# MarcoPolo/drand

Measured on AMD Instinct MI355X. Metric: verified beacons/sec (whole node), quicknet G1 scheme, higher is better.
Workload: dtype u32 (Fp products on 14x28-bit limbs, 64-bit MAD accumulators; 12x32-bit Montgomery storage); 1 GPU; bls-unchained-g1-rfc9380 batch verify of a 1048576-round chain, 1048576 rounds per GPU; scheme=bls-unchained-g1-rfc9380, rounds_total=1048576, rounds_per_gpu=1048576, global_batch=1048576, parallelism=round-shard x1

## Files before the change

### drand_amd/_lib.py

```python
import ctypes
import os

HERE = os.path.dirname(os.path.abspath(__file__))
LIB_PATH = os.environ.get("DRANDHIP_LIB") or os.path.join(HERE, "libdrandhip.so")

DH_OK = 0
DH_EINVAL = -1
DH_EDEVICE = -2
DH_ENOMEM = -3
DH_EKEY = -4
DH_ERECOVER = -5
DH_EBUSY = -6
DH_EABANDONED = -7
DH_ECORRUPT = -8
DH_ENOBEACON = -9
DH_NODE_CHECKED = 2
DH_DEFERRED = 1
DH_STORE_TRIMMED, DH_STORE_UNTRIMMED, DH_STORE_AUTO = 0, 1, 2

_c = ctypes
_P = _c.c_void_p
SIGNATURES = {
    "dh_init": (_c.c_int, [_c.c_uint32]),
    "dh_shutdown": (None, []),
    "dh_scheme_from_name": (_c.c_int, [_c.c_char_p]),
    "dh_sig_len": (_c.c_int, [_c.c_int]),
    "dh_key_len": (_c.c_int, [_c.c_int]),
    "dh_verify_batch": (_c.c_int, [_c.c_int, _c.c_char_p, _c.c_size_t, _P, _P, _c.c_size_t, _P, _c.c_size_t, _P,
                                   _c.c_size_t, _P, _P, _c.c_uint64]),
    "dh_verify_batch_device": (_c.c_int, [_c.c_int, _c.c_char_p, _c.c_size_t, _P, _P, _c.c_size_t, _P, _c.c_size_t,
                                          _P, _c.c_size_t, _P, _P, _c.c_uint64, _P, _P]),
    "dh_verify_beacon": (_c.c_int, [_c.c_int, _c.c_char_p, _c.c_size_t, _c.c_uint64, _c.c_char_p, _c.c_size_t,
                                    _c.c_char_p, _c.c_size_t]),
    "dh_verify_recovered": (_c.c_int, [_c.c_int, _c.c_char_p, _c.c_size_t, _c.c_char_p, _c.c_char_p, _c.c_size_t]),
    "dh_verify_recovered_batch": (_c.c_int, [_c.c_int, _c.c_char_p, _c.c_size_t, _P, _P, _c.c_size_t, _c.c_size_t, _P,
                                             _c.c_uint64]),
    "dh_digest_batch": (_c.c_int, [_c.c_int, _P, _P, _c.c_size_t, _P, _c.c_size_t, _P]),
    "dh_randomness_batch": (_c.c_int, [_c.c_int, _P, _c.c_size_t, _c.c_size_t, _P]),
    "dh_recover_batch": (_c.c_int, [_c.c_int, _c.c_char_p, _c.c_int, _c.c_int, _P, _P, _P, _c.c_size_t, _P, _P]),
    "dh_verify_partials_batch": (_c.c_int, [_c.c_int, _c.c_char_p, _c.c_int, _c.c_int, _P, _P, _P, _c.c_size_t, _P]),
    "dh_bls_verify_batch": (_c.c_int, [_c.c_int, _P, _c.c_size_t, _P, _P, _P, _P, _c.c_size_t, _c.c_size_t, _P, _P,
                                       _c.c_uint64, _P]),
    "dh_identity_hash_batch": (_c.c_int, [_c.c_int, _P, _c.c_size_t, _P]),
    "dh_identity_verify_batch": (_c.c_int, [_c.c_int, _P, _P, _c.c_size_t, _c.c_size_t, _P]),
    "dh_schnorr_verify_batch": (_c.c_int, [_c.c_int, _P, _c.c_size_t, _P, _P, _P, _P, _c.c_size_t, _c.c_size_t, _P, _P]),
    "dh_schnorr_sig_len": (_c.c_int, [_c.c_int]),
    "dh_sign_batch": (_c.c_int, [_c.c_int, _c.c_char_p, _P, _P, _c.c_size_t, _P, _c.c_size_t, _P]),
    "dh_public_key": (_c.c_int, [_c.c_int, _c.c_char_p, _P]),
    "dh_partial_bytes": (_c.c_int, [_c.c_int]),
    "dh_set_split": (_c.c_int, [_c.c_uint64, _c.c_int]),
    "dh_hash_to_curve": (_c.c_int, [_c.c_int, _P, _P, _c.c_size_t, _c.c_char_p, _c.c_size_t, _P]),
    "dh_batch_begin": (_c.c_int, [_c.c_int, _c.c_char_p, _c.c_size_t, _P, _P, _c.c_size_t, _P, _c.c_size_t, _P,
                                  _c.c_size_t, _P, _P, _c.c_uint64, _P, _c.POINTER(_P), _P]),
    "dh_batch_check": (_c.c_int, [_P, _P, _c.c_size_t, _P]),
    "dh_batch_stream": (_P, [_P]),
    "dh_check_partials": (_c.c_int, [_c.c_int, _c.c_char_p, _c.c_size_t, _P, _c.c_size_t, _c.POINTER(_c.c_int)]),
    "dh_batch_finish": (_c.c_int, [_P, _c.c_int, _P]),
    "dh_bolt_index": (_c.c_int, [_P, _c.c_size_t, _P, _P, _c.c_size_t, _P]),
    "dh_store_open_bolt": (_c.c_int, [_P, _c.c_size_t, _c.POINTER(_P)]),
    "dh_store_stat": (_c.c_int, [_P, _P]),
    "dh_store_columns_device": (_c.c_int, [_P, _c.c_uint64, _c.c_uint64, _c.c_size_t, _P, _P, _P, _c.c_size_t, _P, _P,
                                           _c.c_size_t, _P, _P]),
    "dh_store_check_past": (_c.c_int, [_P, _c.c_int, _c.c_char_p, _c.c_size_t, _c.c_uint64, _c.c_size_t, _c.c_uint64, _P,
                                       _c.c_size_t, _P, _P, _P]),
    "dh_store_close": (None, [_P]),
    "dh_store_open_bolt_format": (_c.c_int, [_P, _c.c_size_t, _c.c_int, _c.POINTER(_P)]),
    "dh_store_format_stat": (_c.c_int, [_P, _P]),
    "dh_store_beacons_device": (_c.c_int, [_P, _c.c_uint64, _c.c_uint64, _c.c_size_t, _c.c_size_t, _P, _P, _P, _P, _P, _P,
                                           _c.c_size_t, _P, _P, _c.c_size_t, _P, _P]),
    "dh_store_deferred": (_c.c_int, [_P, _c.c_uint64, _c.c_uint64, _P, _c.c_size_t, _P]),
    "dh_profile": (_c.c_int, [_c.c_int]),
    "dh_profile_read": (_c.c_int, [_c.c_char_p, _c.c_size_t]),
    "dh_last_error_string": (_c.c_char_p, []),
    "dh_version": (_c.c_char_p, []),
}

_lib = None


class LibraryMissing(RuntimeError):
    pass


def load():
# ... 18 lines not shown
```

### drand_amd/csrc/codec.hpp

```cpp
#pragma once
#include "h2c.hpp"
#include "fp28.hpp"
#include "fp2_28.hpp"

namespace dh {

enum : uint8_t { DEC_OK = 1, DEC_INF = 2, DEC_BAD = 0 };

DH_DEV bool fp_lex_gt_half(const fp& mont_y) { return int_gt_half_p(fp_from_mont(mont_y)); }

DH_DEV bool fp2_lex_largest(const fp2& y) {
  fp c0 = fp_from_mont(y.c0), c1 = fp_from_mont(y.c1);
  return fp_is_zero(c1) ? int_gt_half_p(c0) : int_gt_half_p(c1);
}

DH_DEV void be48_words(uint32_t out[12], const uint8_t* in, bool mask_flags) {
#pragma unroll
  for (int i = 0; i < 12; i++) {
    uint32_t w = __builtin_bswap32(*(const uint32_t*)(in + 44 - 4 * i));
    out[i] = w;
  }
  if (mask_flags) out[11] &= 0x1fffffffu;
}

DH_DEV bool g1_in_subgroup(const aff<fp>& p) {
  return g1_in_subgroup28([&] { return p; });
}

DH_DEV bool g2_in_subgroup(const aff<fp2>& p) {
  return g2_in_subgroup28(p);
}

DH_DEV uint8_t g1_decompress(aff<fp>& out, const uint8_t* b, bool subgroup) {
  uint32_t w[12];
  be48_words(w, b, false);
  const uint32_t flags = w[11] >> 29;
  if (!(flags & 4)) return DEC_BAD;
  w[11] &= 0x1fffffffu;
  if (flags & 2) {
    uint32_t nz = flags & 1;
#pragma unroll
    for (int i = 0; i < 12; i++) nz |= w[i];
    return nz ? DEC_BAD : DEC_INF;
  }
  if (!int_lt_p(w)) return DEC_BAD;
  fp x;
#pragma unroll
  for (int i = 0; i < 12; i++) x.v[i] = w[i];
  x = fp_to_mont(x);
  fp rhs = fp_add(fp_mul(fp_sqr(x), x), fp_c(cst::B1));
  fp y;
  if (!fp_sqrt(y, rhs)) return DEC_BAD;
  if (fp_lex_gt_half(y) != (bool)(flags & 1)) y = fp_neg(y);
  out.x = x;
  out.y = y;
  if (subgroup && !g1_in_subgroup(out)) return DEC_BAD;
  return DEC_OK;
}

DH_DEV uint8_t g2_decompress(aff<fp2>& out, const uint8_t* b, bool subgroup) {
  uint32_t w1[12], w0[12];
  be48_words(w1, b, false);
  be48_words(w0, b + 48, false);
  const uint32_t flags = w1[11] >> 29;
  if (!(flags & 4)) return DEC_BAD;
  w1[11] &= 0x1fffffffu;
  if (flags & 2) {
    uint32_t nz = flags & 1;
#pragma unroll
    for (int i = 0; i < 12; i++) nz |= w1[i] | w0[i];
    return nz ? DEC_BAD : DEC_INF;
  }
  if (!int_lt_p(w0) || !int_lt_p(w1)) return DEC_BAD;
  fp2 x;
#pragma unroll
  for (int i = 0; i < 12; i++) {
    x.c0.v[i] = w0[i];
    x.c1.v[i] = w1[i];
  }
  x.c0 = fp_to_mont(x.c0);
  x.c1 = fp_to_mont(x.c1);
  fp2 rhs = fp2_add(fp2_mul(fp2_sqr(x), x), fp2_c(cst::B2));
  fp2 y;
  if (!fp2_sqrt(y, rhs)) return DEC_BAD;
  if (fp2_lex_largest(y) != (bool)(flags & 1)) y = fp2_neg(y);
  out.x = x;
  out.y = y;
  if (subgroup && !g2_in_subgroup(out)) return DEC_BAD;
  return DEC_OK;
// ... 36 lines not shown
```

### drand_amd/csrc/drandhip.cpp

```cpp
#include <hip/hip_runtime.h>
#include <stdarg.h>
#include <stdio.h>
#include <string.h>
#include <sys/random.h>

#include <algorithm>
#include <atomic>
#include <condition_variable>
#include <cmath>
#include <functional>
#include <map>
#include <memory>
#include <chrono>
#include <mutex>
#include <string>
#include <thread>
#include <vector>

#include "../../include/drandhip.h"
#include "bolt.hpp"
#include "kernels.hpp"

namespace {

// ... 711 lines not shown
static bool subgroup_batch_on() {
  static const bool v = [] {
    const char* e = getenv("DRANDHIP_SUBGROUP_BATCH");
    return !(e && e[0] == '0');
  }();
  return v;
}
static size_t sub_batch_min() {
  static const size_t v = [] {
    const char* e = getenv("DRANDHIP_SUB_BATCH_MIN");
    const long long d = e ? atoll(e) : 0;
    return (size_t)(d >= 1 ? d : 131072);
  }();
  return v;
}
constexpr size_t SUB_BATCH_MIN_G2_DEFAULT = 393216;
static size_t sub_batch_min_g2() {
  static const size_t v = [] {
    const char* e = getenv("DRANDHIP_SUB_BATCH_MIN_G2");
    const long long d = e ? atoll(e) : 0;
    return (size_t)(d >= 1 ? d : SUB_BATCH_MIN_G2_DEFAULT);
  }();
  return v;
}
static int sub_backoff() {
  static const int v = [] {
    const char* e = getenv("DRANDHIP_SUB_BACKOFF");
    const long d = e ? atol(e) : -1;
    return (int)(d >= 0 && d <= 1 << 20 ? d : 15);
  }();
  return v;
}

static int msm_workspace(worker* w, const dh::msm_geom& g, size_t m, size_t ngroups, size_t jw, dh::msm_ws& ws,
                         bool sub = false, bool g2 = false) {
  const size_t nk = ngroups * g.nwin * (size_t)g.nbuck;
  HIP_TRY(w->cnt.ensure(nk * 4));
  HIP_TRY(w->off.ensure((nk + 1) * 4));
  HIP_TRY(w->scan_tmp.ensure(((nk + 4095) / 4096 + 1) * 4));
  HIP_TRY(w->list.ensure(dh::msm_entries(g, m) * 4));
  HIP_TRY(w->buckets.ensure(2 * nk * jw * 4));
  const size_t segs_bytes = 2 * ngroups * g.nwin * g.nseg * jw * 4;
  HIP_TRY(w->segs.ensure(2 * segs_bytes));
  HIP_TRY(w->outA.ensure(ngroups * jw * 4));
  HIP_TRY(w->outB.ensure(ngroups * jw * 4));
  HIP_TRY(w->out2.ensure(2 * ngroups * jw * 4));
  HIP_TRY(w->pass.ensure(ngroups));
  HIP_TRY(w->part.ensure(dh::msm_part_bytes(dh::msm_entries(g, m), jw, 2)));
  HIP_TRY(w->meta.ensure(dh::msm_meta_bytes(dh::msm_entries(g, m))));
  ws = dh::msm_ws{w->cnt.as<uint32_t>(), w->off.as<uint32_t>(), w->scan_tmp.as<uint32_t>(), w->list.as<uint32_t>(),
                  w->buckets.as<uint32_t>(), w->segs.as<uint32_t>(), w->out2.as<uint32_t>(), w->part.as<uint32_t>(),
                  w->meta.as<uint32_t>(), 0, (uint32_t*)((uint8_t*)w->segs.p + segs_bytes)};
  if (sub) {
    HIP_TRY(w->sub_tmp.ensure(dh::sub_batch_tmp_bytes(g2, g)));
    HIP_TRY(w->sub_pass.ensure(8));
    ws.sub = w->sub_tmp.as<uint32_t>();
  }
  return DH_OK;
}

int verify_core(worker* w, int scheme, const uint8_t* pk, size_t pk_len, const uint64_t* d_rounds, const uint8_t* d_sigs,
                size_t sig_stride, const uint8_t* d_prevs, size_t prev_stride, const uint32_t* d_prev_lens, size_t n,
                uint8_t* d_verdict, uint8_t* d_rand, uint64_t seed, hipStream_t st, uint64_t* stats,
                const uint8_t* d_msgs32 = nullptr, int mode = VM_FULL, prep_gate* gate = nullptr) {
  const bool g2 = sig_on_g2(scheme);
  const int sig_len = g2 ? 96 : 48, key_len = g2 ? 48 : 96;
// ... 13 lines not shown
                            subgroup_batch_on();
  const bool sub_batch = sub_eligible && w->sub_fused_left == 0;
  if (sub_eligible && w->sub_fused_left > 0) w->sub_fused_left--;
  const int parts = g2 && !sub_batch ? 4 : 2;
  if (n >= ((size_t)1 << 31) / parts) return fail(DH_EINVAL, "batch too large");
  dh::msm_geom g0{};
  dh::msm_ws ws0{};
  if (mode <= VM_BEGIN) {
    int rc = ensure_key(w, g2, pk, pk_len, st);
    if (rc) return rc;

    HIP_TRY(w->status.ensure(n));
    HIP_TRY(w->sig_aff.ensure(n * aw * 4));
    HIP_TRY(w->q_pts.ensure(n * jw * 4));
    HIP_TRY(w->scal.ensure(n * 16));
    HIP_TRY(w->entries.ensure(n * 4));
    uint32_t seedw[8];
    rc = make_seed(seed, seedw);
    if (rc) return rc;
    uint32_t* d_seed = (uint32_t*)((uint8_t*)w->key_ok.p + 32);
    presorted = w->tail && st == w->stream && !skip0 && !one_stream;
    if (presorted) {
      hipStream_t ts = w->tail;
      HIP_TRY(hipMemcpyAsync(d_seed, seedw, 32, hipMemcpyHostToDevice, ts));
      HIP_TRY(dh::launch_scalars(d_seed, n, nullptr, w->scal.as<uint4>(), parts, ts));
      HIP_TRY(dh::launch_iota(w->entries.as<uint32_t>(), n, ts));
      g0 = geom_for(n, parts);
      g0.half_stride = (uint32_t)n;
      rc = msm_workspace(w, g0, n, 1, wsw, ws0, sub_batch, g2);
      if (rc) return rc;
      HIP_TRY(dh::launch_msm_sort(g0, w->entries.as<uint32_t>(), nullptr, nullptr, n, 1, w->scal.as<uint4>(), ws0, ts));
    }
    if (gate && gate->wait) HIP_TRY(hipStreamWaitEvent(st, gate->wait, 0));
    HIP_TRY(T.run(g2 ? "k_prep_sig<fp2>" : "k_prep_sig<fp>", [&] {
      return dh::launch_prep(g2, d_sigs, sig_stride, n, w->status.as<uint8_t>(), w->sig_aff.as<uint32_t>(), d_rand, st,
                             sub_batch);
    }));
    HIP_TRY(w->h2c_tmp.ensure(dh::hash_tmp_bytes(g2, n)));
    HIP_TRY(T.run(d_msgs32 ? (g2 ? "k_prep_msg32<fp2>" : "k_prep_msg32<fp>") : (g2 ? "k_prep_msg<fp2>" : "k_prep_msg<fp>"), [&] {
      return dh::launch_hash(g2, d_rounds, d_prevs, prev_stride, d_prev_lens, d_msgs32, n,
                             scheme == DH_SCHEME_CHAINED && d_prevs && !d_msgs32 ? 1 : 0, dst_id(scheme), w->status.as<uint8_t>(),
                             w->q_pts.as<uint32_t>(), w->h2c_tmp.as<uint32_t>(), st);
    }));
    if (!presorted) {
      HIP_TRY(hipMemcpyAsync(d_seed, seedw, 32, hipMemcpyHostToDevice, st));
      HIP_TRY(dh::launch_scalars(d_seed, n, w->status.as<uint8_t>(), w->scal.as<uint4>(), parts, st));
    }
    HIP_TRY(w->s28.ensure(parts * n * (g2 ? 64 : 32) * 4));
    HIP_TRY(w->q28.ensure(parts * n * (g2 ? 64 : 32) * 4));
    HIP_TRY(T.run(g2 ? "k_msm_prep28<fp2>" : "k_msm_prep28<fp>", [&] {
      return dh::launch_msm_prep28(g2, n, w->status.as<uint8_t>(), w->sig_aff.as<uint32_t>(), w->q_pts.as<uint32_t>(),
                                   w->s28.as<uint32_t>(), w->q28.as<uint32_t>(), st, 3, parts);
    }));
    HIP_TRY(hipMemsetAsync(d_verdict, 0, n, st));
    if (gate) {
      HIP_TRY(hipEventRecord(gate->done, st));
      gate->recorded();
    }
    if (mode == VM_FULL && w->tail && st == w->stream && !one_stream && prep_sync()) HIP_TRY(hipStreamSynchronize(st));
    if (!presorted) HIP_TRY(dh::launch_iota(w->entries.as<uint32_t>(), n, st));
  }
  if (w->tail && st == w->stream && !one_stream) {
    if (mode <= VM_BEGIN) {
      HIP_TRY(hipEventRecord(w->handoff, st));
      HIP_TRY(hipStreamWaitEvent(w->tail, w->handoff, 0));
    }
    st = w->tail;
    T.st = st;
  }

  size_t m = n;
  static const char* const msm_names[8] = {"msm_level0", "msm_bisect1", "msm_bisect2", "msm_bisect3",
                                           "msm_bisect4", "msm_bisect5", "msm_bisect6", "msm_bisect7+"};
  static const char* const chk_names[8] = {"k_group_check_level0", "k_group_check_bisect1", "k_group_check_bisect2",
                                           "k_group_check_bisect3", "k_group_check_bisect4", "k_group_check_bisect5",
                                           "k_group_check_bisect6", "k_group_check_bisect7+"};
// ... 1522 lines not shown
  if (n == 0) return DH_OK;
  size_t maxm = 0;
  for (size_t i = 0; i < n; i++) {
    if (msg_off[i + 1] < msg_off[i]) return fail(DH_EINVAL, "msg_off must be non-decreasing");
    maxm = std::max<size_t>(maxm, msg_off[i + 1] - msg_off[i]);
  }
  const size_t total = msg_off[n] - msg_off[0];
  const size_t stride = (64 + maxm + 4 + dst_len + 63) & ~(size_t)63;
  const size_t outlen = group == 1 ? 48 : 96;
  std::vector<uint32_t> off(n + 1);
  for (size_t i = 0; i <= n; i++) off[i] = msg_off[i] - msg_off[0];
  lease L;
  if (L.rc) return L.rc;
  worker* w = L.w;
  int rc = set_device_and_stream(w);
  if (rc) return rc;
  hipStream_t st = w->stream;
  HIP_TRY(w->in_sigs.ensure(total + 4));
  HIP_TRY(w->in_prev_lens.ensure((n + 1) * 4));
  HIP_TRY(w->key_raw.ensure(256));
  HIP_TRY(w->h2c_tmp.ensure(n * stride));
  HIP_TRY(w->out_rand.ensure(n * outlen));
  if (total) HIP_TRY(hipMemcpyAsync(w->in_sigs.p, msgs + msg_off[0], total, hipMemcpyHostToDevice, st));
  HIP_TRY(hipMemcpyAsync(w->in_prev_lens.p, off.data(), (n + 1) * 4, hipMemcpyHostToDevice, st));
  HIP_TRY(hipMemcpyAsync(w->key_raw.p, dst, dst_len, hipMemcpyHostToDevice, st));
  HIP_TRY(dh::launch_h2c_generic(group == 2, w->in_sigs.as<uint8_t>(), w->in_prev_lens.as<uint32_t>(), n,
                                 w->key_raw.as<uint8_t>(), (uint32_t)dst_len, w->h2c_tmp.as<uint8_t>(), stride,
                                 w->out_rand.as<uint8_t>(), st));
  HIP_TRY(hipMemcpyAsync(out, w->out_rand.p, n * outlen, hipMemcpyDeviceToHost, st));
  HIP_TRY(hipStreamSynchronize(st));
  return DH_OK;
}

int dh_public_key(int scheme, const uint8_t* sk32, uint8_t* key_out) {
  int kl = dh_key_len(scheme);
  if (kl < 0) return kl;
  if (!sk32 || !key_out) return fail(DH_EINVAL, "null argument");
  lease L;
  if (L.rc) return L.rc;
  worker* w = L.w;
  int rc = set_device_and_stream(w);
  if (rc) return rc;
  hipStream_t st = w->stream;
  uint32_t skw[8];
  sk_words(sk32, skw);
  HIP_TRY(w->key_ok.ensure(64));
  HIP_TRY(w->key_raw.ensure(96));
  HIP_TRY(hipMemcpyAsync(w->key_ok.p, skw, 32, hipMemcpyHostToDevice, st));
  HIP_TRY(dh::launch_pubkey(kl == 96, w->key_ok.as<uint32_t>(), w->key_raw.as<uint8_t>(), st));
  HIP_TRY(hipMemcpyAsync(key_out, w->key_raw.p, kl, hipMemcpyDeviceToHost, st));
  HIP_TRY(hipStreamSynchronize(st));
  return DH_OK;
}

}


static size_t store_max_bytes() {
  const char* e = getenv("DRANDHIP_STORE_MAX_BYTES");
  const long long v = e ? atoll(e) : 0;
  return v > 0 ? (size_t)v : (size_t)16 << 30;
}

struct prof_wall {
  const char* name;
  std::chrono::steady_clock::time_point t0;
// ... 647 lines not shown
```

### drand_amd/csrc/h2c.hpp

```cpp
#pragma once
#include "curve.hpp"
#include "sha256.hpp"
#include "fp28.hpp"

namespace dh {

DH_DEV fp fp_from_be512(const uint32_t hi[8], const uint32_t lo[8]) {
  fp h, l;
#pragma unroll
  for (int k = 0; k < 8; k++) {
    h.v[k] = hi[7 - k];
    l.v[k] = lo[7 - k];
  }
#pragma unroll
  for (int k = 8; k < 12; k++) h.v[k] = l.v[k] = 0;
  return fp_add(fp_mul(h, fp_c(cst::K256R)), fp_mul(l, fp_c(cst::R2)));
}

DH_DEV bool fp_sqrt_ratio(fp& y, const fp& u, const fp& v) {
  fp tv1 = fp_sqr(v);
  fp tv2 = fp_mul(u, v);
  tv1 = fp_mul(tv1, tv2);
  fp y1 = fp_pow_sched(tv1, cst::SCHED_SR1_C1, cst::SCHED_SR1_C1_LEN);
  y1 = fp_mul(y1, tv2);
// ... 64 lines not shown
  r.x = f_mul(s.xn, s.xd);
  r.y = f_mul(s.y, f_mul(f_sqr(s.xd), s.xd));
  return r;
}

template <class F>
DH_DEV bool jac_add_distinct(jac<F>& r, const jac<F>& p, const jac<F>& q) {
  F z1z1 = f_sqr(p.z);
  F z2z2 = f_sqr(q.z);
  F u1 = f_mul(p.x, z2z2);
  F u2 = f_mul(q.x, z1z1);
  F s1 = f_mul(f_mul(p.y, q.z), z2z2);
  F s2 = f_mul(f_mul(q.y, p.z), z1z1);
  F h = f_sub(u2, u1);
  if (f_is_zero(h)) return false;
  F rr = f_dbl(f_sub(s2, s1));
  F i = f_sqr(f_dbl(h));
  F j = f_mul(h, i);
  F v = f_mul(u1, i);
  r.x = f_sub(f_sub(f_sqr(rr), j), f_dbl(v));
  r.y = f_sub(f_mul(rr, f_sub(v, r.x)), f_dbl(f_mul(s1, j)));
  r.z = f_mul(f_sub(f_sub(f_sqr(f_add(p.z, q.z)), z1z1), z2z2), h);
  return true;
}

DH_DEV jac<fp> h2c_g1_map(const fp& u0, const fp& u1) {
  const jac<fp> p0 = swu_jac(sswu_g1(u0));
  const jac<fp> p1 = swu_jac(sswu_g1(u1));
  jac<fp> s;
  if (jac_add_distinct(s, p0, p1)) return iso11_jac(s);
  return jac_add(iso11_jac(p0), iso11_jac(p1));
}

DH_DEV jac<fp> h2c_g1_noclear(const sha_h& digest, int dst_id) {
  uint32_t b[4][8];
  xmd32<4>(b, digest, dst_id);
  return h2c_g1_map(fp_from_be512(b[0], b[1]), fp_from_be512(b[2], b[3]));
}

DH_DEV jac<fp> h2c_clear_g1(const jac<fp>& p) { return jac_add(jac_mul_uabs_j(p), p); }

DH_DEV swu_out<fp2> sswu_g2(const fp2& u) {
  const fp2 A = fp2_c(cst::SSWU2_A), B = fp2_c(cst::SSWU2_B), Z = fp2_c(cst::SSWU2_Z);
  fp2 tv1 = fp2_mul(Z, fp2_sqr(u));
  fp2 tv2 = fp2_add(fp2_sqr(tv1), tv1);
  fp2 tv3 = fp2_mul(B, fp2_add(tv2, fp2_one()));
  fp2 tv4 = fp2_mul(A, fp2_select(fp2_is_zero(tv2), Z, fp2_neg(tv2)));
  fp2 t2 = fp2_sqr(tv3);
  fp2 tv6 = fp2_sqr(tv4);
  t2 = fp2_add(t2, fp2_mul(A, tv6));
  t2 = fp2_mul(t2, tv3);
  tv6 = fp2_mul(tv6, tv4);
  t2 = fp2_add(t2, fp2_mul(B, tv6));
  fp2 x = fp2_mul(tv1, tv3);
  fp2 y1;
  bool gx1_sq = fp2_sqrt_ratio_cm(y1, t2, tv6);
  fp2 y = fp2_mul(fp2_mul(tv1, u), y1);
  x = fp2_select(gx1_sq, tv3, x);
  y = fp2_select(gx1_sq, y1, y);
  bool e1 = fp2_sgn0(u) == fp2_sgn0(y);
  y = fp2_select(e1, y, fp2_neg(y));
  return {x, tv4, y};
}

DH_DEV jac<fp2> iso3_jac(const jac<fp2>& p) {
  using namespace cst;
// ... 58 lines not shown
```

### drand_amd/csrc/k_prep.hip

```cpp
#include "kcommon.hpp"

namespace dh {

template <class F>
__global__ __launch_bounds__(256, occ<F>::W) void k_prep_sig(const uint8_t* __restrict__ sigs, size_t stride, size_t n,
                                                  uint8_t* __restrict__ status, uint32_t* __restrict__ sig_aff,
                                                  uint8_t* __restrict__ rand_out) {
  size_t i = gtid();
  if (i >= n) return;
  const uint8_t* s = sigs + i * stride;
  aff<F> a;
  uint8_t st;
  if constexpr (sizeof(F) == sizeof(fp)) {
    st = g1_decompress(a, s, false);
    if (st == DEC_OK) st_aff_aos<F>(sig_aff, i, a);
    if (rand_out) st_digest(rand_out + 32 * i, sha256_aligned<48>(s));
    if (st == DEC_OK && !g1_in_subgroup28([&] { return ld_aff_aos<fp>(sig_aff, i); })) st = DEC_BAD;
    if (st == DEC_OK) {
      status[i] = st;
      return;
    }
  } else {
    st = g2_decompress(a, s, true);
    if (rand_out) st_digest(rand_out + 32 * i, sha256_aligned<96>(s));
// ... 152 lines not shown
}

hipError_t launch_dec_sig(int sig_g2, const uint8_t* sigs, size_t stride, size_t n, uint8_t* status, uint32_t* sig_aff,
                          uint8_t* rand_out, hipStream_t st) {
  if (!n) return hipSuccess;
  if (sig_g2)
    hipLaunchKernelGGL(k_dec_sig_g2, dim3(nblk(n, 256)), dim3(256), 0, st, sigs, stride, n, status, sig_aff, rand_out);
  else
    hipLaunchKernelGGL(k_dec_sig_g1, dim3(nblk(n, 64)), dim3(64), 0, st, sigs, stride, n, status, sig_aff, rand_out);
  return hipGetLastError();
}

hipError_t launch_sub_flag(int sig_g2, size_t n, const uint8_t* status, const uint32_t* sig_aff, uint8_t* sub_bad, hipStream_t st) {
  if (!n) return hipSuccess;
  if (sig_g2) hipLaunchKernelGGL(k_sub_flag<fp2>, dim3(nblk(n, 64)), dim3(64), 0, st, n, status, sig_aff, sub_bad);
  else hipLaunchKernelGGL(k_sub_flag<fp>, dim3(nblk(n, 64)), dim3(64), 0, st, n, status, sig_aff, sub_bad);
  return hipGetLastError();
}

hipError_t launch_and_subgroup(size_t n, const uint8_t* sub_bad, uint8_t* verdict, hipStream_t st) {
  if (!n) return hipSuccess;
  hipLaunchKernelGGL(k_and_subgroup, dim3(nblk(n, 64)), dim3(64), 0, st, n, sub_bad, verdict);
  return hipGetLastError();
}

__global__ __launch_bounds__(256, occ<fp>::W) void k_prep_msg_g1(const uint64_t* __restrict__ rounds, const uint8_t* __restrict__ prevs,
                                                            size_t prev_stride, const uint32_t* __restrict__ prev_lens,
                                                            const uint8_t* __restrict__ msgs32, size_t n, int chained, int dst_id,
                                                            uint8_t* __restrict__ status, uint32_t* __restrict__ q_out) {
  size_t i = gtid();
  if (i >= n) return;
  const sha_h d = message_of(rounds, prevs, prev_stride, prev_lens, msgs32, chained, i, status);
  st_jac_aos<fp>(q_out, i, h2c_g1_noclear(d, dst_id));
}

__global__ __launch_bounds__(256) void k_h2f_g2(const uint64_t* __restrict__ rounds, const uint8_t* __restrict__ prevs,
                                                size_t prev_stride, const uint32_t* __restrict__ prev_lens,
                                                const uint8_t* __restrict__ msgs32, size_t n, int chained, int dst_id,
                                                uint8_t* __restrict__ status, uint32_t* __restrict__ u_out) {
  size_t i = gtid();
  if (i >= n) return;
  const sha_h d = message_of(rounds, prevs, prev_stride, prev_lens, msgs32, chained, i, status);
  uint32_t b[8][8];
  xmd32<8>(b, d, dst_id);
  const fp2 u0 = {fp_from_be512(b[0], b[1]), fp_from_be512(b[2], b[3])};
  const fp2 u1 = {fp_from_be512(b[4], b[5]), fp_from_be512(b[6], b[7])};
  st_f<fp2>(u_out + 48 * i, u0);
  st_f<fp2>(u_out + 48 * i + 24, u1);
}

__global__ __launch_bounds__(256, 2) void k_sswu_g2(const uint32_t* __restrict__ u, size_t m, uint32_t* __restrict__ pts) {
  size_t j = gtid();
  if (j >= m) return;
  fp2 x;
  ld_f<fp2>(x, u + 24 * j);
  st_jac_aos<fp2>(pts, j, swu_jac(sswu_g2(x)));
}

__global__ __launch_bounds__(256, 2) void k_add_iso_g2(const uint32_t* __restrict__ pts, size_t n, uint32_t* __restrict__ q_out,
                                                       uint32_t* __restrict__ exc) {
  size_t i = gtid();
  if (i >= n) return;
  jac<fp2> s;
  if (!jac_add_distinct_mem(s, pts + 144 * i, pts + 144 * i + 72)) {
    exc[1 + atomicAdd(exc, 1u)] = (uint32_t)i;
    return;
// ... 141 lines not shown
hipError_t launch_decode_key(int key_g2, const uint8_t* pk, uint32_t* key_aff, uint8_t* ok, hipStream_t st) {
  if (key_g2) hipLaunchKernelGGL(k_decode_key<fp2>, dim3(1), dim3(128), 0, st, pk, key_aff, ok);
  else hipLaunchKernelGGL(k_decode_key<fp>, dim3(1), dim3(128), 0, st, pk, key_aff, ok);
  return hipGetLastError();
}


size_t hash_tmp_bytes(int sig_g2, size_t n) { return sig_g2 ? n * 2 * 72 * 4 + (n + 1) * 4 : 0; }

static hipError_t hash_g2_map(size_t n, uint32_t* q_out, uint32_t* tmp, hipStream_t st) {
  hipLaunchKernelGGL(k_sswu_g2, dim3(nblk(2 * n, 256)), dim3(256), 0, st, (const uint32_t*)q_out, 2 * n, tmp);
  uint32_t* exc = tmp + n * 2 * 72;
  hipError_t e = hipMemsetAsync(exc, 0, 4, st);
  if (e != hipSuccess) return e;
  hipLaunchKernelGGL(k_add_iso_g2, dim3(nblk(n, 256)), dim3(256), 0, st, (const uint32_t*)tmp, n, q_out, exc);
  hipLaunchKernelGGL(k_add_iso_g2_exc, dim3(1), dim3(EXC_THREADS), 0, st, (const uint32_t*)tmp, (const uint32_t*)exc, q_out);
  return hipGetLastError();
}

hipError_t launch_hash(int sig_g2, const uint64_t* rounds, const uint8_t* prevs, size_t prev_stride, const uint32_t* prev_lens,
                       const uint8_t* msgs32, size_t n, int chained, int dst_id, uint8_t* status, uint32_t* q_out, uint32_t* tmp,
                       hipStream_t st) {
  if (!n) return hipSuccess;
  if (!sig_g2) {
    hipLaunchKernelGGL(k_prep_msg_g1, dim3(nblk(n, 256)), dim3(256), 0, st, rounds, prevs, prev_stride, prev_lens, msgs32, n,
                       chained, dst_id, status, q_out);
    return hipGetLastError();
  }
  hipLaunchKernelGGL(k_h2f_g2, dim3(nblk(n, 256)), dim3(256), 0, st, rounds, prevs, prev_stride, prev_lens, msgs32, n, chained,
                     dst_id, status, q_out);
  return hash_g2_map(n, q_out, tmp, st);
}

hipError_t launch_hash_var(int sig_g2, const uint8_t* msgs, const uint32_t* msg_off, size_t n, int dst_id, uint32_t* q_out,
                           uint32_t* tmp, hipStream_t st) {
  if (!n) return hipSuccess;
  if (!sig_g2) {
    hipLaunchKernelGGL(k_prep_msgv_g1, dim3(nblk(n, 256)), dim3(256), 0, st, msgs, msg_off, n, dst_id, q_out);
    return hipGetLastError();
  }
  hipLaunchKernelGGL(k_h2fv_g2, dim3(nblk(n, 256)), dim3(256), 0, st, msgs, msg_off, n, dst_id, q_out);
  return hash_g2_map(n, q_out, tmp, st);
}

DH_COUNTER_ACCESSOR(prep)

}
```

### drand_amd/csrc/kernels.hpp

```cpp
#pragma once
#include <cstdlib>
#include <hip/hip_runtime.h>
#include <stddef.h>
#include <stdint.h>

namespace dh {

struct msm_geom {
  uint32_t gsize;
  int c;
  int nwin;
  uint32_t nbuck;
  uint32_t nseg;
  uint32_t seglen;
  uint32_t halves;
  uint32_t half_stride;
};
inline size_t msm_entries(const msm_geom& g, size_t m) { return m * (size_t)g.nwin * g.halves; }

struct msm_ws {
  uint32_t* cnt;
  uint32_t* off;
  uint32_t* scan_tmp;
  uint32_t* list;
// ... 8 lines not shown
};

inline uint32_t msm_chunk_len(size_t max_entries, size_t cap = 32, size_t target_chunks = 262144) {
  static const size_t lmin = [] {
    const char* e = getenv("DRANDHIP_MSM_LMIN");
    const long v = e ? atol(e) : 0;
    return (size_t)(v >= 1 && v <= 64 ? v : 8);
  }();
  size_t L = max_entries / target_chunks;
  if (L < lmin) L = lmin;
  return (uint32_t)(L > cap ? cap : L);
}
inline size_t msm_nchunks(size_t max_entries) { return max_entries / msm_chunk_len(max_entries) + 2; }
inline size_t msm_part_bytes(size_t max_entries, size_t jac_words, int nsets) {
  return msm_nchunks(max_entries) * 2 * jac_words * 4 * (size_t)nsets;
}
inline size_t msm_meta_bytes(size_t max_entries) { return msm_nchunks(max_entries) * 2 * 4; }

hipError_t launch_prep(int sig_g2, const uint8_t* sigs, size_t stride, size_t n, uint8_t* status, uint32_t* sig_aff,
                       uint8_t* rand_out, hipStream_t st, bool defer_sub = false);
hipError_t launch_sub_exact(int sig_g2, size_t n, uint8_t* status, uint32_t* sig_aff, uint8_t* sub_bad, uint32_t* nbad, hipStream_t st);
hipError_t launch_dec_sig(int sig_g2, const uint8_t* sigs, size_t stride, size_t n, uint8_t* status, uint32_t* sig_aff,
                          uint8_t* rand_out, hipStream_t st);
hipError_t launch_sub_flag(int sig_g2, size_t n, const uint8_t* status, const uint32_t* sig_aff, uint8_t* sub_bad, hipStream_t st);
hipError_t launch_and_subgroup(size_t n, const uint8_t* sub_bad, uint8_t* verdict, hipStream_t st);
size_t hash_small_tmp_bytes(int sig_g2, size_t n);
hipError_t launch_hash_small(int sig_g2, const uint64_t* rounds, const uint8_t* prevs, size_t prev_stride, const uint32_t* prev_lens,
                             const uint8_t* msgs32, size_t n, int chained, int dst_id, uint8_t* status, uint32_t* q_out,
                             uint32_t* tmp, hipStream_t st);
size_t hash_tmp_bytes(int sig_g2, size_t n);
hipError_t launch_hash(int sig_g2, const uint64_t* rounds, const uint8_t* prevs, size_t prev_stride, const uint32_t* prev_lens,
                       const uint8_t* msgs32, size_t n, int chained, int dst_id, uint8_t* status, uint32_t* q_out, uint32_t* tmp,
                       hipStream_t st);
hipError_t launch_hash_var(int sig_g2, const uint8_t* msgs, const uint32_t* msg_off, size_t n, int dst_id, uint32_t* q_out,
                           uint32_t* tmp, hipStream_t st);
hipError_t launch_scalars(const uint32_t* seed_words, size_t n, const uint8_t* status, uint4* scal, int parts, hipStream_t st);
hipError_t launch_decode_key(int key_g2, const uint8_t* pk, uint32_t* key_aff, uint8_t* ok, hipStream_t st);
hipError_t launch_iota(uint32_t* v, size_t n, hipStream_t st);
hipError_t launch_scan(const uint32_t* cnt, size_t nk, uint32_t* off, uint32_t* tmp, hipStream_t st);
hipError_t launch_msm_prep28(int sig_g2, size_t n, uint8_t* status, const uint32_t* sig_aff, const uint32_t* q_pts,
                             uint32_t* S, uint32_t* Q, hipStream_t st, uint32_t sets = 3, int parts = 0);
hipError_t launch_msm28_set(int sig_g2, const msm_geom& g, const uint32_t* pidx, const uint32_t* sidx, const uint32_t* grp,
                            size_t m, size_t ngroups, const uint4* scal, const uint32_t* P, msm_ws& ws, uint32_t* out,
                            hipStream_t st);
hipError_t launch_msm28(int sig_g2, const msm_geom& g, const uint32_t* entries, size_t m, size_t ngroups, const uint4* scal,
                        const uint32_t* S, const uint32_t* Q, msm_ws& ws, uint32_t* outA, uint32_t* outB, hipStream_t st,
                        const uint8_t* skip, bool presorted);
size_t sub_batch_tmp_bytes(int sig_g2, const msm_geom& g);
hipError_t launch_sub_batch(int sig_g2, const msm_geom& g, const msm_ws& ws, uint8_t* pass, uint8_t* sub_pass, hipStream_t st);
hipError_t launch_msm_sort(const msm_geom& g, const uint32_t* pidx, const uint32_t* sidx, const uint32_t* grp, size_t m,
                           size_t ngroups, const uint4* scal, msm_ws& ws, hipStream_t st);
hipError_t launch_group_check(int sig_g2, const uint32_t* A, const uint32_t* B, size_t ngroups, const uint32_t* key_aff,
                              uint8_t* pass, hipStream_t st);
hipError_t launch_sum_partials(int sig_g2, const uint32_t* parts, size_t k, size_t rec_words, uint32_t* outA, uint32_t* outB,
                               uint8_t* flag, hipStream_t st);
hipError_t launch_node_mark(size_t n, uint8_t* res, const uint8_t* status, uint8_t* verdict, hipStream_t st);
hipError_t launch_mark_groups(const uint32_t* entries, size_t m, size_t gsize, const uint8_t* pass, const uint8_t* status,
                              uint8_t* verdict, hipStream_t st);
hipError_t launch_compact_failing(const uint32_t* entries, size_t m, size_t gsize, size_t ngroups, const uint8_t* pass,
                                  uint32_t* flags, uint32_t* rank, uint32_t* scan_tmp, uint32_t* out, hipStream_t st);
hipError_t launch_leaf_check(int sig_g2, const uint32_t* entries, size_t m, const uint32_t* sig_aff, const uint32_t* q_pts,
                             const uint32_t* key_aff, const uint8_t* status, uint8_t* verdict, hipStream_t st);

hipError_t launch_group_check_vm(int sig_g2, const uint32_t* A, const uint32_t* B, size_t ngroups, const uint32_t* key_aff,
                                 const uint32_t* key_h,
                                 uint32_t* pairs, uint8_t* live, uint8_t* pass, hipStream_t st);
// ... 111 lines not shown
```

### include/drandhip.h

```cpp
#ifndef DRANDHIP_H
#define DRANDHIP_H

#include <stddef.h>
#include <stdint.h>

#ifdef __cplusplus
extern "C" {
#endif

#define DH_OK 0
#define DH_EINVAL (-1)
#define DH_EDEVICE (-2)
#define DH_ENOMEM (-3)
#define DH_EKEY (-4)
#define DH_ERECOVER (-5)
#define DH_EBUSY (-6)
#define DH_EABANDONED (-7)
#define DH_ECORRUPT (-8)
#define DH_ENOBEACON (-9)

#define DH_SCHEME_CHAINED 0
#define DH_SCHEME_UNCHAINED 1
#define DH_SCHEME_G1_LEGACY 2
#define DH_SCHEME_G1_RFC9380 3
// ... 66 lines not shown
int dh_bolt_index(const uint8_t* file, size_t len, uint32_t* page_size_out, uint64_t* leaf_off_out, size_t cap,
                  size_t* n_leaves_out);

typedef struct dh_store dh_store;
int dh_store_open_bolt(const uint8_t* file, size_t len, dh_store** out);
int dh_store_stat(const dh_store* store, uint64_t out[6]);
int dh_store_columns_device(dh_store* store, uint64_t first, uint64_t last, size_t row_stride, uint64_t* d_rounds,
                            uint8_t* d_rows, uint32_t* d_lens, size_t cap_rows, size_t* n_rows_out, uint64_t* d_missing,
                            size_t cap_missing, size_t* n_missing_out, void* hip_stream);
int dh_store_check_past(dh_store* store, int scheme, const uint8_t* pk, size_t pk_len, uint64_t up_to, size_t window,
                        uint64_t seed, uint64_t* faulty_out, size_t cap, size_t* n_faulty_out,
                        void (*cb)(uint64_t round, uint64_t up_to, void* arg), void* cb_arg);
void dh_store_close(dh_store* store);

#define DH_STORE_TRIMMED 0
#define DH_STORE_UNTRIMMED 1
#define DH_STORE_AUTO 2
#define DH_DEFERRED 1
int dh_store_open_bolt_format(const uint8_t* file, size_t len, int format, dh_store** out);
int dh_store_format_stat(const dh_store* store, uint64_t out[4]);
int dh_store_beacons_device(dh_store* store, uint64_t first, uint64_t last, size_t sig_stride, size_t prev_stride,
                            uint64_t* d_rounds, uint8_t* d_sigs, uint32_t* d_sig_lens, uint8_t* d_prevs, uint32_t* d_prev_lens,
                            uint8_t* d_deferred, size_t cap_rows, size_t* n_rows_out, uint64_t* d_missing, size_t cap_missing,
                            size_t* n_missing_out, void* hip_stream);
int dh_store_deferred(dh_store* store, uint64_t first, uint64_t last, uint64_t* out, size_t cap, size_t* n_out);

int dh_sign_batch(int scheme, const uint8_t* sk32, const uint64_t* rounds, const uint8_t* prevs, size_t n,
                  const uint32_t* prev_lens, size_t prev_stride, uint8_t* sigs_out);
int dh_public_key(int scheme, const uint8_t* sk32, uint8_t* key_out);

int dh_hash_to_curve(int group, const uint8_t* msgs, const uint32_t* msg_off, size_t n, const uint8_t* dst, size_t dst_len,
                     uint8_t* out);

int dh_profile(int enable);
int dh_profile_read(char* buf, size_t cap);

const char* dh_last_error_string(void);

const char* dh_version(void);

#ifdef __cplusplus
}
#endif
#endif
```

Baseline: 47.02 million beacons/s.

## Fuse G1 signature decompression with hash-to-curve sharing one exponentiation for inversion

Adds a fused per-round G1 kernel that hashes the message, maps both field elements through SSWU, and decompresses the signature in one launch. The signature square root is rearranged so the same exponentiation also yields the inverse needed for the affine addition of the two mapped points (a Montgomery-style trick). The isogeny is then applied to an affine point, which avoids a separate field inversion and a second kernel launch with its temporary buffer. It is enabled by default for G1 sub-batches. It adds branch-free paths for invalid inputs and a fallback for coincident mapped points.

```diff
diff --git a/drand_amd/_lib.py b/drand_amd/_lib.py
--- a/drand_amd/_lib.py
+++ b/drand_amd/_lib.py
@@ -50,6 +50,7 @@
     "dh_partial_bytes": (_c.c_int, [_c.c_int]),
     "dh_set_split": (_c.c_int, [_c.c_uint64, _c.c_int]),
     "dh_hash_to_curve": (_c.c_int, [_c.c_int, _P, _P, _c.c_size_t, _c.c_char_p, _c.c_size_t, _P]),
+    "dh_g1_round_prep_debug": (_c.c_int, [_P, _P, _c.c_size_t, _P, _P, _P]),
     "dh_batch_begin": (_c.c_int, [_c.c_int, _c.c_char_p, _c.c_size_t, _P, _P, _c.c_size_t, _P, _c.c_size_t, _P,
                                   _c.c_size_t, _P, _P, _c.c_uint64, _P, _c.POINTER(_P), _P]),
     "dh_batch_check": (_c.c_int, [_P, _P, _c.c_size_t, _P]),
diff --git a/drand_amd/csrc/codec.hpp b/drand_amd/csrc/codec.hpp
--- a/drand_amd/csrc/codec.hpp
+++ b/drand_amd/csrc/codec.hpp
@@ -55,6 +55,30 @@
   out.x = x;
   out.y = y;
   if (subgroup && !g1_in_subgroup(out)) return DEC_BAD;
+  return DEC_OK;
+}
+
+DH_DEV uint8_t g1_decompress_ride(aff<fp>& out, fp& inv_c, const uint8_t* b, const fp& c) {
+  uint32_t w[12];
+  be48_words(w, b, false);
+  const uint32_t flags = w[11] >> 29;
+  w[11] &= 0x1fffffffu;
+  uint32_t nz = flags & 1;
+#pragma unroll
+  for (int i = 0; i < 12; i++) nz |= w[i];
+  const uint8_t pre = !(flags & 4) ? DEC_BAD : (flags & 2) ? (nz ? DEC_BAD : DEC_INF) : int_lt_p(w) ? DEC_OK : DEC_BAD;
+  fp x;
+#pragma unroll
+  for (int i = 0; i < 12; i++) x.v[i] = pre == DEC_OK ? w[i] : 0;
+  x = fp_to_mont(x);
+  const fp rhs = fp_select(pre == DEC_OK, fp_add(fp_mul(fp_sqr(x), x), fp_c(cst::B1)), fp_one());
+  fp y;
+  const bool qr = fp_sqrt_ride(y, inv_c, rhs, c);
+  if (pre != DEC_OK) return pre;
+  if (!qr) return DEC_BAD;
+  if (fp_lex_gt_half(y) != (bool)(flags & 1)) y = fp_neg(y);
+  out.x = x;
+  out.y = y;
   return DEC_OK;
 }
 
diff --git a/drand_amd/csrc/drandhip.cpp b/drand_amd/csrc/drandhip.cpp
--- a/drand_amd/csrc/drandhip.cpp
+++ b/drand_amd/csrc/drandhip.cpp
@@ -767,6 +767,14 @@
   return v;
 }
 
+static bool g1_ride_on() {
+  static const bool v = [] {
+    const char* e = getenv("DRANDHIP_G1_RIDE");
+    return !(e && e[0] == '0');
+  }();
+  return v;
+}
+
 static int msm_workspace(worker* w, const dh::msm_geom& g, size_t m, size_t ngroups, size_t jw, dh::msm_ws& ws,
                          bool sub = false, bool g2 = false) {
   const size_t nk = ngroups * g.nwin * (size_t)g.nbuck;
@@ -846,16 +854,24 @@
       HIP_TRY(dh::launch_msm_sort(g0, w->entries.as<uint32_t>(), nullptr, nullptr, n, 1, w->scal.as<uint4>(), ws0, ts));
     }
     if (gate && gate->wait) HIP_TRY(hipStreamWaitEvent(st, gate->wait, 0));
-    HIP_TRY(T.run(g2 ? "k_prep_sig<fp2>" : "k_prep_sig<fp>", [&] {
-      return dh::launch_prep(g2, d_sigs, sig_stride, n, w->status.as<uint8_t>(), w->sig_aff.as<uint32_t>(), d_rand, st,
-                             sub_batch);
-    }));
-    HIP_TRY(w->h2c_tmp.ensure(dh::hash_tmp_bytes(g2, n)));
-    HIP_TRY(T.run(d_msgs32 ? (g2 ? "k_prep_msg32<fp2>" : "k_prep_msg32<fp>") : (g2 ? "k_prep_msg<fp2>" : "k_prep_msg<fp>"), [&] {
-      return dh::launch_hash(g2, d_rounds, d_prevs, prev_stride, d_prev_lens, d_msgs32, n,
-                             scheme == DH_SCHEME_CHAINED && d_prevs && !d_msgs32 ? 1 : 0, dst_id(scheme), w->status.as<uint8_t>(),
-                             w->q_pts.as<uint32_t>(), w->h2c_tmp.as<uint32_t>(), st);
-    }));
+    const int chained = scheme == DH_SCHEME_CHAINED && d_prevs && !d_msgs32 ? 1 : 0;
+    if (!g2 && sub_batch && g1_ride_on()) {
+      HIP_TRY(T.run(d_msgs32 ? "k_prep_msg32<fp>" : "k_prep_msg<fp>", [&] {
+        return dh::launch_round_g1_ride(d_rounds, d_prevs, prev_stride, d_prev_lens, d_msgs32, n, chained, dst_id(scheme), d_sigs,
+                                        sig_stride, w->status.as<uint8_t>(), w->sig_aff.as<uint32_t>(), d_rand,
+                                        w->q_pts.as<uint32_t>(), st);
+      }));
+    } else {
+      HIP_TRY(T.run(g2 ? "k_prep_sig<fp2>" : "k_prep_sig<fp>", [&] {
+        return dh::launch_prep(g2, d_sigs, sig_stride, n, w->status.as<uint8_t>(), w->sig_aff.as<uint32_t>(), d_rand, st,
+                               sub_batch);
+      }));
+      HIP_TRY(w->h2c_tmp.ensure(dh::hash_tmp_bytes(g2, n)));
+      HIP_TRY(T.run(d_msgs32 ? (g2 ? "k_prep_msg32<fp2>" : "k_prep_msg32<fp>") : (g2 ? "k_prep_msg<fp2>" : "k_prep_msg<fp>"), [&] {
+        return dh::launch_hash(g2, d_rounds, d_prevs, prev_stride, d_prev_lens, d_msgs32, n, chained, dst_id(scheme),
+                               w->status.as<uint8_t>(), w->q_pts.as<uint32_t>(), w->h2c_tmp.as<uint32_t>(), st);
+      }));
+    }
     if (!presorted) {
       HIP_TRY(hipMemcpyAsync(d_seed, seedw, 32, hipMemcpyHostToDevice, st));
       HIP_TRY(dh::launch_scalars(d_seed, n, w->status.as<uint8_t>(), w->scal.as<uint4>(), parts, st));
@@ -2444,6 +2460,43 @@
   return DH_OK;
 }
 
+static bool fp_bytes_canonical(const uint8_t* b) {
+  static const uint8_t P[48] = {0x1a, 0x01, 0x11, 0xea, 0x39, 0x7f, 0xe6, 0x9a, 0x4b, 0x1b, 0xa7, 0xb6, 0x43, 0x4b, 0xac, 0xd7,
+                                0x64, 0x77, 0x4b, 0x84, 0xf3, 0x85, 0x12, 0xbf, 0x67, 0x30, 0xd2, 0xa0, 0xf6, 0xb0, 0xf6, 0x24,
+                                0x1e, 0xab, 0xff, 0xfe, 0xb1, 0x53, 0xff, 0xff, 0xb9, 0xfe, 0xff, 0xff, 0xff, 0xff, 0xaa, 0xab};
+  return memcmp(b, P, 48) < 0;
+}
+
+int dh_g1_round_prep_debug(const uint8_t* us, const uint8_t* sigs, size_t n, uint8_t* status_out, uint8_t* sig_out,
+                           uint8_t* hash_out) {
+  if (!us || !sigs || !status_out || !sig_out || !hash_out) return fail(DH_EINVAL, "null argument");
+  if (n == 0) return DH_OK;
+  for (size_t i = 0; i < 2 * n; i++)
+    if (!fp_bytes_canonical(us + 48 * i)) return fail(DH_EINVAL, "field element %zu is not below p", i);
+  lease L;
+  if (L.rc) return L.rc;
+  worker* w = L.w;
+  int rc = set_device_and_stream(w);
+  if (rc) return rc;
+  hipStream_t st = w->stream;
+  HIP_TRY(w->in_prevs.ensure(n * 96));
+  HIP_TRY(w->in_sigs.ensure(n * 48));
+  HIP_TRY(w->status.ensure(n));
+  HIP_TRY(w->sig_aff.ensure(n * JAC_WORDS_G1 * 2 / 3 * 4));
+  HIP_TRY(w->q_pts.ensure(n * JAC_WORDS_G1 * 4));
+  HIP_TRY(w->out_rand.ensure(n * 192));
+  HIP_TRY(hipMemcpyAsync(w->in_prevs.p, us, n * 96, hipMemcpyHostToDevice, st));
+  HIP_TRY(hipMemcpyAsync(w->in_sigs.p, sigs, n * 48, hipMemcpyHostToDevice, st));
+  uint8_t* out = w->out_rand.as<uint8_t>();
+  HIP_TRY(dh::launch_round_g1_ride_debug(w->in_prevs.as<uint8_t>(), w->in_sigs.as<uint8_t>(), n, w->status.as<uint8_t>(),
+                                         w->sig_aff.as<uint32_t>(), w->q_pts.as<uint32_t>(), out, out + n * 96, st));
+  HIP_TRY(hipMemcpyAsync(status_out, w->status.p, n, hipMemcpyDeviceToHost, st));
+  HIP_TRY(hipMemcpyAsync(sig_out, out, n * 96, hipMemcpyDeviceToHost, st));
+  HIP_TRY(hipMemcpyAsync(hash_out, out + n * 96, n * 96, hipMemcpyDeviceToHost, st));
+  HIP_TRY(hipStreamSynchronize(st));
+  return DH_OK;
+}
+
 int dh_public_key(int scheme, const uint8_t* sk32, uint8_t* key_out) {
   int kl = dh_key_len(scheme);
   if (kl < 0) return kl;
diff --git a/drand_amd/csrc/h2c.hpp b/drand_amd/csrc/h2c.hpp
--- a/drand_amd/csrc/h2c.hpp
+++ b/drand_amd/csrc/h2c.hpp
@@ -120,6 +120,58 @@
   return jac_add(iso11_jac(p0), iso11_jac(p1));
 }
 
+DH_DEV bool fp_sqrt_ride(fp& y, fp& inv_c, const fp& a, const fp& c) {
+  const fp ac = fp_mul(a, c);
+  const fp w = fp_pow_sched(fp_mul(ac, c), cst::SCHED_SR1_C1, cst::SCHED_SR1_C1_LEN);
+  y = fp_mul(w, ac);
+  const fp ic = fp_mul(fp_sqr(w), ac);
+  const bool qr = fp_eq(fp_sqr(y), a);
+  inv_c = fp_select(qr, ic, fp_neg(ic));
+  return qr;
+}
+
+struct g1_sum_mid {
+  fp n, s, a, dyd2, y0;
+};
+DH_DEV bool g1_sum_pre(g1_sum_mid& m, fp& c, const swu_out<fp>& p0, const swu_out<fp>& p1) {
+  m.a = fp_mul(p0.xn, p1.xd);
+  const fp b = fp_mul(p1.xn, p0.xd);
+  const fp d = fp_mul(p0.xd, p1.xd);
+  m.n = fp_sub(b, m.a);
+  m.s = fp_add(b, m.a);
+  c = fp_mul(m.n, d);
+  m.dyd2 = fp_mul(fp_sub(p1.y, p0.y), fp_sqr(d));
+  m.y0 = p0.y;
+  return !fp_is_zero(m.n);
+}
+DH_DEV aff<fp> g1_sum_post(const g1_sum_mid& m, const fp& inv_c) {
+  const fp inv_d = fp_mul(m.n, inv_c);
+  const fp lam = fp_mul(m.dyd2, inv_c);
+  aff<fp> r;
+  r.x = fp_sub(fp_sqr(lam), fp_mul(m.s, inv_d));
+  r.y = fp_sub(fp_mul(lam, fp_sub(fp_mul(m.a, inv_d), r.x)), m.y0);
+  return r;
+}
+
+DH_DEV jac<fp> iso11_aff(const aff<fp>& p) {
+  using namespace cst;
+  const f28 X = f28_from_fp(p.x);
+  f28 xn = f28_c(ISO11_XNUM_28[ISO11_XNUM_LEN - 1]);
+  f28 yn = f28_c(ISO11_YNUM_28[ISO11_YNUM_LEN - 1]);
+  f28 h = X;
+#pragma unroll 1
+  for (int j = 1; j < ISO11_YNUM_LEN; j++) {
+    yn = f28_add(f28_mul(yn, X), f28_c(ISO11_YNUM_28[ISO11_YNUM_LEN - 1 - j]));
+    if (j < ISO11_XNUM_LEN) xn = f28_add(f28_mul(xn, X), f28_c(ISO11_XNUM_28[ISO11_XNUM_LEN - 1 - j]));
+    if (j < ISO11_H_LEN) h = f28_add(j > 1 ? f28_mul(h, X) : h, f28_c(ISO11_H_28[ISO11_H_LEN - 1 - j]));
+  }
+  jac<fp> r;
+  r.x = f28_to_fp(xn);
+  r.y = f28_to_fp(f28_mul(f28_from_fp(p.y), yn));
+  r.z = f28_to_fp(h);
+  return r;
+}
+
 DH_DEV jac<fp> h2c_g1_noclear(const sha_h& digest, int dst_id) {
   uint32_t b[4][8];
   xmd32<4>(b, digest, dst_id);
diff --git a/drand_amd/csrc/k_prep.hip b/drand_amd/csrc/k_prep.hip
--- a/drand_amd/csrc/k_prep.hip
+++ b/drand_amd/csrc/k_prep.hip
@@ -208,6 +208,82 @@
   if (i >= n) return;
   const sha_h d = message_of(rounds, prevs, prev_stride, prev_lens, msgs32, chained, i, status);
   st_jac_aos<fp>(q_out, i, h2c_g1_noclear(d, dst_id));
+}
+
+DH_DEV void round_g1_ride(const fp& u0, const fp& u1, bool msg_ok, const uint8_t* __restrict__ s, size_t i,
+                          uint8_t* __restrict__ status, uint32_t* __restrict__ sig_aff, uint8_t* __restrict__ rand_out,
+                          uint32_t* __restrict__ q_out) {
+  st_f<fp>(q_out + 36 * i, u0);
+  st_f<fp>(q_out + 36 * i + 12, u1);
+  g1_sum_mid m;
+  fp c;
+  const bool distinct = g1_sum_pre(m, c, sswu_g1(u0), sswu_g1(u1));
+  c = fp_select(distinct, c, fp_one());
+  fp inv_c;
+  {
+    aff<fp> a;
+    uint8_t st = g1_decompress_ride(a, inv_c, s, c);
+    if (rand_out) st_digest(rand_out + 32 * i, sha256_aligned<48>(s));
+    if (st != DEC_OK) {
+      a.x = fp{};
+      a.y = fp{};
+      st = DEC_BAD;
+    }
+    status[i] = msg_ok ? st : (uint8_t)DEC_BAD;
+    st_aff_aos<fp>(sig_aff, i, a);
+  }
+  if (distinct) {
+    st_jac_aos<fp>(q_out, i, iso11_aff(g1_sum_post(m, inv_c)));
+  } else {
+    fp v0, v1;
+    ld_f<fp>(v0, q_out + 36 * i);
+    ld_f<fp>(v1, q_out + 36 * i + 12);
+    st_jac_aos<fp>(q_out, i, h2c_g1_map(v0, v1));
+  }
+}
+
+__global__ __launch_bounds__(256, occ<fp>::W) void k_round_g1_ride(const uint64_t* __restrict__ rounds, const uint8_t* __restrict__ prevs,
+                                                              size_t prev_stride, const uint32_t* __restrict__ prev_lens,
+                                                              const uint8_t* __restrict__ msgs32, size_t n, int chained, int dst_id,
+                                                              const uint8_t* __restrict__ sigs, size_t stride,
+                                                              uint8_t* __restrict__ status, uint32_t* __restrict__ sig_aff,
+                                                              uint8_t* __restrict__ rand_out, uint32_t* __restrict__ q_out) {
+  size_t i = gtid();
+  if (i >= n) return;
+  sha_h d;
+  bool msg_ok = true;
+  if (msgs32) d = message_of(nullptr, nullptr, 0, nullptr, msgs32, 0, i, nullptr);
+  else msg_ok = beacon_digest(d, rounds, prevs, prev_stride, prev_lens, chained, i);
+  uint32_t b[4][8];
+  xmd32<4>(b, d, dst_id);
+  round_g1_ride(fp_from_be512(b[0], b[1]), fp_from_be512(b[2], b[3]), msg_ok, sigs + i * stride, i, status, sig_aff, rand_out,
+                q_out);
+}
+
+__global__ __launch_bounds__(256, occ<fp>::W) void k_round_g1_ride_debug(const uint8_t* __restrict__ u, size_t n,
+                                                                    const uint8_t* __restrict__ sigs, size_t stride,
+                                                                    uint8_t* __restrict__ status, uint32_t* __restrict__ sig_aff,
+                                                                    uint32_t* __restrict__ q_out) {
+  size_t i = gtid();
+  if (i >= n) return;
+  fp u0, u1;
+  be48_words(u0.v, u + 96 * i, false);
+  be48_words(u1.v, u + 96 * i + 48, false);
+  round_g1_ride(fp_to_mont(u0), fp_to_mont(u1), true, sigs + i * stride, i, status, sig_aff, nullptr, q_out);
+}
+__global__ __launch_bounds__(64) void k_round_g1_debug_out(size_t n, const uint32_t* __restrict__ sig_aff,
+                                                           const uint32_t* __restrict__ q_pts, uint8_t* __restrict__ sig_out,
+                                                           uint8_t* __restrict__ q_out) {
+  size_t i = gtid();
+  if (i >= n) return;
+  const aff<fp> s = ld_aff_aos<fp>(sig_aff, i);
+  st_be48(sig_out + 96 * i, fp_from_mont(s.x));
+  st_be48(sig_out + 96 * i + 48, fp_from_mont(s.y));
+  const jac<fp> q = ld_jac_aos<fp>(q_pts, i);
+  aff<fp> a{fp{}, fp{}};
+  if (!jac_is_inf(q)) a = jac_to_aff(q);
+  st_be48(q_out + 96 * i, fp_from_mont(a.x));
+  st_be48(q_out + 96 * i + 48, fp_from_mont(a.y));
 }
 
 __global__ __launch_bounds__(256) void k_h2f_g2(const uint64_t* __restrict__ rounds, const uint8_t* __restrict__ prevs,
@@ -415,6 +491,24 @@
   return hash_g2_map(n, q_out, tmp, st);
 }
 
+hipError_t launch_round_g1_ride(const uint64_t* rounds, const uint8_t* prevs, size_t prev_stride, const uint32_t* prev_lens,
+                                const uint8_t* msgs32, size_t n, int chained, int dst_id, const uint8_t* sigs, size_t stride,
+                                uint8_t* status, uint32_t* sig_aff, uint8_t* rand_out, uint32_t* q_out, hipStream_t st) {
+  if (!n) return hipSuccess;
+  hipLaunchKernelGGL(k_round_g1_ride, dim3(nblk(n, 256)), dim3(256), 0, st, rounds, prevs, prev_stride, prev_lens, msgs32, n,
+                     chained, dst_id, sigs, stride, status, sig_aff, rand_out, q_out);
+  return hipGetLastError();
+}
+
+hipError_t launch_round_g1_ride_debug(const uint8_t* u, const uint8_t* sigs, size_t n, uint8_t* status, uint32_t* sig_aff,
+                                      uint32_t* q_pts, uint8_t* sig_out, uint8_t* q_out, hipStream_t st) {
+  if (!n) return hipSuccess;
+  hipLaunchKernelGGL(k_round_g1_ride_debug, dim3(nblk(n, 256)), dim3(256), 0, st, u, n, sigs, (size_t)48, status, sig_aff, q_pts);
+  hipLaunchKernelGGL(k_round_g1_debug_out, dim3(nblk(n, 64)), dim3(64), 0, st, n, (const uint32_t*)sig_aff,
+                     (const uint32_t*)q_pts, sig_out, q_out);
+  return hipGetLastError();
+}
+
 hipError_t launch_hash_var(int sig_g2, const uint8_t* msgs, const uint32_t* msg_off, size_t n, int dst_id, uint32_t* q_out,
                            uint32_t* tmp, hipStream_t st) {
   if (!n) return hipSuccess;
diff --git a/drand_amd/csrc/kernels.hpp b/drand_amd/csrc/kernels.hpp
--- a/drand_amd/csrc/kernels.hpp
+++ b/drand_amd/csrc/kernels.hpp
@@ -64,6 +64,11 @@
 hipError_t launch_hash(int sig_g2, const uint64_t* rounds, const uint8_t* prevs, size_t prev_stride, const uint32_t* prev_lens,
                        const uint8_t* msgs32, size_t n, int chained, int dst_id, uint8_t* status, uint32_t* q_out, uint32_t* tmp,
                        hipStream_t st);
+hipError_t launch_round_g1_ride(const uint64_t* rounds, const uint8_t* prevs, size_t prev_stride, const uint32_t* prev_lens,
+                                const uint8_t* msgs32, size_t n, int chained, int dst_id, const uint8_t* sigs, size_t stride,
+                                uint8_t* status, uint32_t* sig_aff, uint8_t* rand_out, uint32_t* q_out, hipStream_t st);
+hipError_t launch_round_g1_ride_debug(const uint8_t* u, const uint8_t* sigs, size_t n, uint8_t* status, uint32_t* sig_aff,
+                                      uint32_t* q_pts, uint8_t* sig_out, uint8_t* q_out, hipStream_t st);
 hipError_t launch_hash_var(int sig_g2, const uint8_t* msgs, const uint32_t* msg_off, size_t n, int dst_id, uint32_t* q_out,
                            uint32_t* tmp, hipStream_t st);
 hipError_t launch_scalars(const uint32_t* seed_words, size_t n, const uint8_t* status, uint4* scal, int parts, hipStream_t st);
diff --git a/include/drandhip.h b/include/drandhip.h
--- a/include/drandhip.h
+++ b/include/drandhip.h
@@ -122,6 +122,9 @@
 int dh_hash_to_curve(int group, const uint8_t* msgs, const uint32_t* msg_off, size_t n, const uint8_t* dst, size_t dst_len,
                      uint8_t* out);
 
+int dh_g1_round_prep_debug(const uint8_t* us, const uint8_t* sigs, size_t n, uint8_t* status_out, uint8_t* sig_out,
+                           uint8_t* hash_out);
+
 int dh_profile(int enable);
 int dh_profile_read(char* buf, size_t cap);
 
```

New measurement: 48.50 million beacons/s (median of 6 runs). +3.1%, better.
